# sunshinnnn/DSMnet

Measured on AMD Instinct MI355X. Metric: stereo pairs/sec forward, PSMNet D=192 384×1280, at 1/2/4/8 MI355X, higher is better.
Workload: dtype f32

## Files before the change

### dsmnet_amd/_lib.py

```python
import ctypes
import os

_HERE = os.path.dirname(os.path.abspath(__file__))
LIB_PATH = os.environ.get("DSM_LIB_PATH") or os.path.join(_HERE, "csrc", "libdsmnet_hip.so")

c_int, c_void_p, c_size_t = ctypes.c_int, ctypes.c_void_p, ctypes.c_size_t

DSM_OK = 0
DSM_F32 = 0
DSM_NCDHW, DSM_NDHWC = 0, 1
DSM_CONV_FP32_MFMA, DSM_CONV_COUT1_CHUNKED, DSM_CONV_TM_SHIFT, DSM_CONV_BLOCKS_SHIFT = 1, 2, 4, 16
DSM_CONV_NO_NSPLIT = 4
DSM_CONV_NO_ONCE = 8
DSM_CONV_KSPLIT_SHIFT = 8
DSM_PREC_F32, DSM_PREC_F16, DSM_PREC_F16X2 = 0, 1, 2
DSM_SIM_DOT, DSM_SIM_COSINE = 0, 1
DSM_CORR_BWD_NAIVE = 1


class Bn3dArgs(ctypes.Structure):
    _fields_ = [("y", c_void_p), ("residual", c_void_p), ("out", c_void_p), ("gamma", c_void_p),
                ("beta", c_void_p), ("running_mean", c_void_p), ("running_var", c_void_p),
                ("affine", c_void_p), ("workspace", c_void_p), ("gout", c_void_p), ("dy", c_void_p),
                ("dresidual", c_void_p), ("B", c_int), ("C", c_int),
# ... 138 lines not shown
    "dsm_stage_images_nhwc16": (c_int, [c_void_p] * 3 + [c_int] * 4 + [c_void_p]),
    "dsm_volume_relayout": (c_int, [c_void_p] * 2 + [c_int] * 6 + [c_void_p]),
    "dsm_conv_packed_weight_bytes": (ctypes.c_size_t, [c_int] * 4),
    "dsm_spp_branch_floats": (ctypes.c_size_t, [c_int] * 3),
    "dsm_spp_pool8": (c_int, [c_void_p] * 2 + [c_int] * 3 + [c_void_p]),
    "dsm_spp_branches": (c_int, [c_void_p] * 5 + [c_int] * 3 + [c_void_p]),
    "dsm_spp_concat": (c_int, [c_void_p] * 4 + [c_int] * 3 + [c_void_p] * 2),
    "dsm_warp_abs_error": (c_int, [c_void_p] * 4 + [c_int] * 6 + [ctypes.c_float, c_void_p]),
    "dsm_warp_abs_error_bwd": (c_int, [c_void_p] * 7 + [c_int] * 6 + [ctypes.c_float, c_void_p]),
    "dsm_decoder_cat_bwd": (c_int, [c_void_p] * 6 + [c_int] * 11 + [c_void_p]),
    "dsm_selfsup_workspace_floats": (c_size_t, [ctypes.POINTER(SelfsupItem), c_int]),
    "dsm_selfsup_fwd": (c_int, [ctypes.POINTER(SelfsupItem), c_int, c_int] + [c_void_p] * 4),
    "dsm_selfsup_bwd": (c_int, [ctypes.POINTER(SelfsupItem), c_int, c_int] + [c_void_p] * 4),
    "dsm_selfsup_ext_workspace_floats": (c_size_t, [ctypes.POINTER(SelfsupItem), c_int, c_int]),
    "dsm_selfsup_ext_fwd": (c_int, [ctypes.POINTER(SelfsupItem), ctypes.POINTER(SelfsupExt), c_int, c_int] + [c_void_p] * 4),
    "dsm_selfsup_ext_bwd": (c_int, [ctypes.POINTER(SelfsupItem), ctypes.POINTER(SelfsupExt), c_int, c_int] + [c_void_p] * 4),
    "dsm_selfsup_dyn_fwd": (c_int, [ctypes.POINTER(SelfsupItem), ctypes.POINTER(SelfsupExt), c_int, c_int] + [c_void_p] * 5),
    "dsm_selfsup_dyn_bwd": (c_int, [ctypes.POINTER(SelfsupItem), ctypes.POINTER(SelfsupExt), c_int, c_int] + [c_void_p] * 5),
    "dsm_suploss_workspace_floats": (c_size_t, [c_int] * 5),
    "dsm_suploss_fwd": (c_int, [ctypes.POINTER(SuplossItem), c_int, c_void_p, c_int, c_int, c_int, c_int] + [c_void_p] * 4),
    "dsm_suploss_bwd": (c_int, [ctypes.POINTER(SuplossItem), c_int, c_void_p, c_int, c_int, c_int] + [c_void_p] * 4),
    "dsm_stereo_metrics_workspace_bytes": (c_size_t, [c_int] * 3),
    "dsm_stereo_metrics": (c_int, [ctypes.POINTER(MetricsArgs), c_void_p]),
    "dsm_lr_check": (c_int, [ctypes.POINTER(LrcheckArgs), c_void_p]),
    "dsm_fill_background_workspace_bytes": (c_size_t, [c_int] * 3),
    "dsm_fill_background": (c_int, [c_void_p] * 4 + [c_int] * 3 + [c_void_p]),
    "dsm_stereo_color": (c_int, [c_void_p, c_void_p, ctypes.POINTER(ColorRecord)] + [c_int] * 6 + [c_void_p]),
    "dsm_stereo_spatial": (c_int, [c_void_p, c_void_p, ctypes.POINTER(SpatialRecord)] + [c_int] * 8 + [c_void_p]),
    "dsm_stereo_spatial_raw": (c_int, [c_void_p, c_size_t, ctypes.POINTER(FrameSource), c_void_p,
                                       ctypes.POINTER(SpatialRecord)] + [c_int] * 8 + [c_void_p]),
    "dsm_stereo_spatial_raw_plan": (c_int, [c_void_p, c_size_t, ctypes.POINTER(FrameSource), c_void_p,
                                            ctypes.POINTER(SpatialRecord)] + [c_int] * 8),
    "dsm_concat_conv_fwd": (c_int, [c_void_p] * 5 + [c_size_t] + [c_void_p] * 2 + [c_int] * 9 + [c_void_p]),
}

_lib = None


class DsmnetHipError(RuntimeError):
    pass


def _bind_torch_hip_runtime():
    import torch
    hip = os.path.join(os.path.dirname(torch.__file__), "lib", "libamdhip64.so")
    if os.path.exists(hip):
        ctypes.CDLL(hip, mode=ctypes.RTLD_GLOBAL)


def load():
    global _lib
    if _lib is not None:
        return _lib
    if not os.path.exists(LIB_PATH):
        raise DsmnetHipError(
            "libdsmnet_hip.so not found at %s -- build it with "
            "`python -m dsmnet_amd.csrc.build` (there is no CPU fallback)" % LIB_PATH)
    _bind_torch_hip_runtime()
    lib = ctypes.CDLL(LIB_PATH)
    for name, (res, args) in SIGNATURES.items():
        fn = getattr(lib, name)
        fn.restype = res
        fn.argtypes = args
    if lib.dsm_abi_version() != 7:
        raise DsmnetHipError("libdsmnet_hip.so ABI version mismatch")
    _lib = lib
# ... 8 lines not shown
```

### dsmnet_amd/blocks2d.py

```python
import torch
import torch.nn as nn
import torch.nn.functional as F

from . import costvolume as cv
from . import blocks3d
from .folds import _bump_running_stats, _versions, fold_affine

_TRAIN_2D_MODE = __import__("os").environ.get("DSM_TRAIN_2D", "auto")
_FUSED_TRAIN_2D = _TRAIN_2D_MODE in ("auto", "fused", "conv")
_FUSED_TRAIN_2D_BN = _TRAIN_2D_MODE == "fused"
_TRAIN_2D_MIN_PIXELS = int(__import__("os").environ.get("DSM_TRAIN_2D_MIN_PIXELS", 65536)) if _TRAIN_2D_MODE == "auto" else 0


class own_kernels_only(object):

    def __enter__(self):
        global _TRAIN_2D_MIN_PIXELS, _FUSED_TRAIN_2D
        self.saved = (_TRAIN_2D_MIN_PIXELS, _FUSED_TRAIN_2D)
        _TRAIN_2D_MIN_PIXELS, _FUSED_TRAIN_2D = 0, True
        return self

    def __exit__(self, *exc):
        global _TRAIN_2D_MIN_PIXELS, _FUSED_TRAIN_2D
        _TRAIN_2D_MIN_PIXELS, _FUSED_TRAIN_2D = self.saved
# ... 56 lines not shown
    if not (cv.get_option("wide_conv2d_train") and isinstance(act, nn.ReLU) and isinstance(conv, nn.Conv2d) and
            x.is_cuda and x.dtype == torch.float32):
        return False
    k, s, d, p = conv.kernel_size, conv.stride, conv.dilation, conv.padding
    if k != (3, 3) or s[0] != s[1] or s[0] not in (1, 2) or d != (1, 1) or p != (1, 1) or conv.groups != 1:
        return False
    if conv.bias is None or conv.padding_mode != "zeros" or conv.weight.dtype != torch.float32:
        return False
    if conv.in_channels not in cv.WIDE2D_COUT or conv.out_channels not in cv.WIDE2D_COUT:
        return False
    B, _, H, W = x.shape
    Ho, Wo = (H - 1) // s[0] + 1, (W - 1) // s[0] + 1
    if W > 2032 or B * H * W >= 2 ** 20 or 4 * B * Ho * Wo * conv.out_channels >= 2 ** 31:
        return False
    return _wide_ok(conv, x)


class _Folded2d(object):
    def __init__(self):
        self.key = None
        self.packed = self.scale = self.shift = None

    def get(self, conv, bn, cin_padded):
        srcs = [conv.weight, conv.bias]
        if bn is not None:
            srcs += [bn.weight, bn.bias, bn.running_mean, bn.running_var]
        key = _versions(*srcs) + (cin_padded,)
        if key != self.key:
            with torch.no_grad():
                self.packed = cv.pack_conv2d_weight(conv.weight, cin_padded)
                self.scale, self.shift = fold_affine(conv.bias, bn, conv.out_channels, conv.weight.device)
            self.key = key
        return self.packed, self.scale, self.shift


def train_ok(conv, x):
    if not (_FUSED_TRAIN_2D and isinstance(conv, nn.Conv2d) and torch.is_tensor(x) and x.is_cuda and
            x.dtype == torch.float32 and conv.weight.dtype == torch.float32):
        return False
    k, s, d, p = conv.kernel_size, conv.stride, conv.dilation, conv.padding
    if k[0] != k[1] or s[0] != s[1] or d[0] != d[1] or p[0] != p[1] or conv.groups != 1:
        return False
    if conv.bias is not None or conv.padding_mode != "zeros" or p[0] != d[0] * (k[0] // 2):
        return False
    if x.shape[0] * ((x.shape[2] - 1) // s[0] + 1) * ((x.shape[3] - 1) // s[0] + 1) < _TRAIN_2D_MIN_PIXELS:
        return False
    return x.shape[1] == conv.in_channels and cv.conv2d_variant(conv.out_channels, s[0], k[0], d[0])


def _run_conv2d_autograd(conv, bn, x, residual, relu):
    y = cv.conv2d(x, conv.weight, conv.stride[0], conv.dilation[0])
    if (bn is not None and bn.training and _FUSED_TRAIN_2D_BN and blocks3d._FUSED_TRAIN_BN and
            y.shape[1] % 4 == 0 and y.shape[1] <= 256):
        momentum = bn.momentum if bn.momentum is not None else 0.1
        out = cv.bn_add_relu2d(y, bn.weight, bn.bias, residual,
                               bn.running_mean if bn.track_running_stats else None,
                               bn.running_var if bn.track_running_stats else None,
                               1 if relu else 0, momentum, bn.eps)
        if bn.num_batches_tracked is not None:
            bn.num_batches_tracked += 1
        _bump_running_stats(bn)
        return out
    if bn is not None:
        y = bn(y)
    if residual is not None:
        y = y + residual
# ... 53 lines not shown
```

### dsmnet_amd/costvolume.py

```python
import collections
import ctypes
import functools
import os
import weakref

import torch

from . import _lib
from .folds import _versions

_CL3D = torch.channels_last_3d


class LaunchTimer(object):

    def __init__(self):
        self.records = []

    def start(self):
        ev = torch.cuda.Event(enable_timing=True)
        ev.record()
        return ev

    def stop(self, name, start, work):
# ... 401 lines not shown
            setattr(a, field, 16)
    buf = ctypes.create_string_buffer(96)
    rc = _lib.load().dsm_conv3d_plan(ctypes.byref(a), buf, 96)
    return rc, buf.value.decode()


_PRECISIONS = ("bf16x3", "fp32", "f16x2", "f16")


def _env_precision():
    v = os.environ.get("DSM_CONV_PRECISION", "")
    if v and v not in _PRECISIONS:
        raise ValueError("DSM_CONV_PRECISION must be one of %s, got %r" % (_PRECISIONS, v))
    return v or "f16x2"


def _env_flag(name, default):
    v = os.environ.get(name, "")
    if v not in ("", "0", "1"):
        raise ValueError("%s must be 0 or 1, got %r" % (name, v))
    return default if v == "" else v == "1"


_WIDE_CONV2D_DEFAULT = False

_OPTIONS = {"fuse_volume": True, "fuse_blocks": True, "conv_precision": _env_precision(), "conv_flags": 0,
            "separable_volume": _env_flag("DSM_SEPARABLE_VOLUME", True), "separable_flags": 0,
            "fused_supervised_loss": _env_flag("DSM_FUSED_SUP_LOSS", True),
            "wide_conv2d": _env_flag("DSM_WIDE_CONV2D", _WIDE_CONV2D_DEFAULT),
            "wide_conv2d_train": _env_flag("DSM_WIDE_CONV2D_TRAIN", False),
            "conv2d_k5": _env_flag("DSM_CONV2D_K5", False),
            "warp_train": _env_flag("DSM_WARP_TRAIN", False),
            "decoder_train": _env_flag("DSM_DECODER_TRAIN", False),
            "corr1d_tiled_bwd": False}


def set_option(name, value):
    if name == "conv_fp32":
        old = _OPTIONS["conv_precision"] == "fp32"
        _OPTIONS["conv_precision"] = "fp32" if value else "bf16x3"
        return old
    if name not in _OPTIONS:
        raise KeyError(name)
    old = _OPTIONS[name]
    if name == "conv_precision":
        if value not in _PRECISIONS:
            raise ValueError("conv_precision must be one of %s" % (_PRECISIONS,))
        _OPTIONS[name] = value
    else:
        _OPTIONS[name] = int(value) if name in ("conv_flags", "separable_flags") else bool(value)
    return old


def _mode(mode):
    return _OPTIONS["conv_precision"] if mode is None else mode


def _conv_flags(mode=None):
    return (_lib.DSM_CONV_FP32_MFMA if _mode(mode) == "fp32" else 0) | _OPTIONS["conv_flags"]


def get_option(name):
    if name == "conv_fp32":
        return _OPTIONS["conv_precision"] == "fp32"
    return _OPTIONS[name]

# ... 623 lines not shown
        if needs_amax():
            dy._dsm_amax = _ARENA.slot(y.device)
            a.dy_amax = dy._dsm_amax.data_ptr()
            if dres is not None:
                dres._dsm_amax = _ARENA.slot(y.device)
                a.dres_amax = dres._dsm_amax.data_ptr()
        with torch.cuda.device(y.device), _timed("bn3d_train_bwd_kernels", 4.0 * (3 * y.numel() + gout.numel())):
            rc = _lib.load().dsm_bn3d_train_bwd(ctypes.byref(a), _stream())
        _lib.check(rc, "dsm_bn3d_train_bwd")
        dbeta = ws[:C].float() if has_beta else None
        dgamma = ws[C:].float() if has_gamma else None
        return dy, dgamma, dbeta, dres, None, None, None, None, None


def bn_add_relu3d(y, gamma, beta, residual, running_mean, running_var, relu, momentum, eps):
    return BnAddRelu3dFunction.apply(y, gamma, beta, residual, running_mean, running_var, int(relu),
                                     float(momentum), float(eps))


def stage_images_nhwc16(left, right=None):
    _require_device("stage_images_nhwc16", left, right)
    left = left.contiguous()
    B, C, H, W = left.shape
    if right is not None:
        if tuple(right.shape) != tuple(left.shape):
            raise ValueError("stage_images_nhwc16: the two views differ in shape")
        right = right.contiguous()
    out = torch.empty(((1 if right is None else 2) * B, 16, H, W), device=left.device,
                      dtype=torch.float32, memory_format=_CL2D)
    with torch.cuda.device(left.device):
        rc = _lib.load().dsm_stage_images_nhwc16(_p(left), _p(right), _p(out), B, C, H, W, _stream())
    _lib.check(rc, "dsm_stage_images_nhwc16")
    return out


def conv2d_variant(cout, stride, k, dilation):
    if cout not in (32, 64, 128) or k not in (1, 3) or stride < 1 or dilation < 1:
        return False
    return _conv2d_variant(cout, stride, k, dilation, _mode(None), _conv_flags())


@functools.lru_cache(maxsize=None)
def _conv2d_variant(cout, stride, k, dilation, mode, flags):
    return _conv_plan(_conv2d_standin(1, 16, cout, 12, 40, stride, k, dilation, mode, flags))[0] == _lib.DSM_OK


def _wgrad2d(x_cl, g_cl, stride, dilation, label="conv2d_wgrad_kernel", mode=None):
    B, cx, Hx, Wx = x_cl.shape
    _, cg, Hg, Wg = g_cl.shape
    ws = torch.empty((cx // 32) * (cg // 32) * 9 * 1024, device=x_cl.device, dtype=torch.float32)
    dw = torch.empty((cg, cx, 3, 3), device=x_cl.device, dtype=torch.float32)
    prec, xa, ga = _wgrad_precision(x_cl, g_cl, mode)
    with torch.cuda.device(x_cl.device), _timed(label, 18.0 * cx * cg * B * Hg * Wg):
        rc = _lib.load().dsm_conv2d_wgrad(_p(x_cl), _p(g_cl), _p(ws), _p(dw), B, cx, cg, Hx, Wx,
                                          Hg, Wg, int(stride), int(dilation), _conv_flags(mode), prec,
                                          _p(xa), _p(ga), _stream())
    _lib.check(rc, "dsm_conv2d_wgrad")
    return dw


class Conv2dFunction(torch.autograd.Function):

    @staticmethod
    def forward(ctx, x, weight, stride, dilation):
        _require_device("Conv2dFunction", x, weight)
        cout, cin, k, _ = weight.shape
# ... 785 lines not shown
```

### dsmnet_amd/csrc/build.py

```python
import glob
import os
import subprocess
import sys
from concurrent.futures import ThreadPoolExecutor

HERE = os.path.dirname(os.path.abspath(__file__))
SOURCES = ["abi.hip", "corr1d.hip", "cost_volume.hip", "soft_argmin.hip", "conv3d.hip", "conv_f16.hip",
           "conv3d_bwd.hip", "bn3d.hip", "decoder.hip", "spp.hip", "warp.hip",
           "selfsup.hip", "color.hip", "spatial.hip", "frames.hip", "sepvol.hip", "suploss.hip", "relu_bwd.hip",
           "metrics.hip", "lrcheck.hip"]
LIB = os.path.join(HERE, "libdsmnet_hip.so")
HIPCC = os.environ.get("HIPCC", "/opt/rocm/bin/hipcc")
FLAGS = ["--offload-arch=gfx950", "-O3", "-std=c++17", "-fPIC",
         "-Wall", "-Wno-unused-function"] + os.environ.get("HIPCC_EXTRA", "").split()


def _stale(out, deps):
    if not os.path.exists(out):
        return True
    t = os.path.getmtime(out)
    return any(os.path.getmtime(d) > t for d in deps)


def build(force=False, verbose=True, stamps=False):
    if stamps:
        lib = os.path.join(HERE, "libdsmnet_hip_stamps.so")
        srcs = [os.path.join(HERE, s) for s in SOURCES]
        extra = ["-DDSM_ABLATE=%s" % os.environ["DSM_ABLATE"]] if os.environ.get("DSM_ABLATE") else []
        cmd = [HIPCC] + FLAGS + ["-DDSM_STAMPS"] + extra + ["-shared", "-o", lib] + srcs
        print(" ".join(cmd), flush=True)
        subprocess.run(cmd, check=True)
        return lib
    hdrs = sorted(glob.glob(os.path.join(HERE, "*.hpp"))) + [os.path.join(HERE, "..", "..", "include", "dsmnet_hip.h")]
    srcs = [os.path.join(HERE, s) for s in SOURCES if os.path.exists(os.path.join(HERE, s))]
    objs = []
    jobs = []
    for s in srcs:
        o = s[:-4] + ".o"
        objs.append(o)
        if force or _stale(o, [s] + hdrs):
            jobs.append([HIPCC] + FLAGS + ["-c", s, "-o", o])

    def run(cmd):
# ... 18 lines not shown
```

### dsmnet_amd/models/psmnet/stackhourglass.py

```python
import math

import torch
import torch.nn as nn

from ... import costvolume as cv
from ...blocks3d import Chain3d, ConvBN3d
from .submodule import convbn_3d, disparityregression, feature_extraction


def myadd_3d(tensor1, tensor2):
    assert tensor1.dim() == 5
    d, h, w = (min(a, b) for a, b in zip(tensor1.shape[2:], tensor2.shape[2:]))
    return tensor1[:, :, :d, :h, :w] + tensor2[:, :, :d, :h, :w]


def _deconvbn_3d(cin, cout):
    return ConvBN3d(nn.ConvTranspose3d(cin, cout, kernel_size=3, padding=1, output_padding=1,
                                       stride=2, bias=False), nn.BatchNorm3d(cout))


class hourglass(nn.Module):
    def __init__(self, inplanes):
        super(hourglass, self).__init__()
        c = inplanes
# ... 18 lines not shown
        super(PSMNet, self).__init__()
        self.name = "psmnet"
        self.maxdisp = maxdisp
        self.align_corners = bool(align_corners)
        self.count_levels = 1
        self.feature_extraction = feature_extraction(align_corners=align_corners)
        relu = lambda: nn.ReLU(inplace=True)
        self.dres0 = Chain3d(convbn_3d(64, 32, 3, 1, 1), relu(), convbn_3d(32, 32, 3, 1, 1), relu())
        self.dres1 = Chain3d(convbn_3d(32, 32, 3, 1, 1), relu(), convbn_3d(32, 32, 3, 1, 1))
        self.dres2 = hourglass(32)
        self.dres3 = hourglass(32)
        self.dres4 = hourglass(32)
        for i in (1, 2, 3):
            setattr(self, "classif%d" % i, Chain3d(
                convbn_3d(32, 32, 3, 1, 1), relu(),
                nn.Conv3d(32, 1, kernel_size=3, padding=1, stride=1, bias=False)))
        self._init_weights()

    def _init_weights(self):
        for m in self.modules():
            if isinstance(m, (nn.Conv2d, nn.Conv3d)):
                fan = m.out_channels
                for k in m.kernel_size:
                    fan *= k
                m.weight.data.normal_(0, math.sqrt(2.0 / fan))
            elif isinstance(m, (nn.BatchNorm2d, nn.BatchNorm3d)):
                m.weight.data.fill_(1)
                m.bias.data.zero_()

    def features(self, left, right):
        if self.training:
            return self.feature_extraction(left), self.feature_extraction(right)
        fe = self.feature_extraction
        if left.is_cuda and not torch.is_grad_enabled() and left.shape[1] <= 16:
            both = fe(cv.stage_images_nhwc16(left, right), staged=True)
        else:
            both = self.feature_extraction(torch.cat([left, right], dim=0))
        self.__dict__["_both"] = both
        return (cv.carry_amax(both[: left.shape[0]], both), cv.carry_amax(both[left.shape[0]:], both))

    def regularise(self, cost):
        cost0 = self.dres0(cost)
        cost0 = self.dres1(cost0, residual=cost0)
        out1, pre1, post1 = self.dres2(cost0, None, None, skip=cost0)
        out2, pre2, post2 = self.dres3(out1, pre1, post1, skip=cost0)
        out3, pre3, post3 = self.dres4(out2, pre1, post2, skip=cost0)
        cost1 = self.classif1(out1)
        cost2 = self.classif2(out2, residual=cost1)
        cost3 = self.classif3(out3, residual=cost2)
        return cost1, cost2, cost3

    def forward(self, left, right, mode="train"):
        with cv.amax_scope(left.device):
            return self._forward(left, right)

    def _forward(self, left, right):
        self.__dict__["_both"] = None
        refimg_fea, targetimg_fea = self.features(left, right)
        both = self.__dict__.pop("_both")
        if (both is not None and cv.get_option("fuse_volume") and not torch.is_grad_enabled() and
                cv.virtual_volume_ok(both.shape[1])):
            cost = cv.VirtualVolume(both, self.maxdisp // 4, True)
        else:
            cost = cv.concat_volume(refimg_fea, targetimg_fea, self.maxdisp // 4, mask_left=True)
        size = (self.maxdisp, left.shape[2], left.shape[3])
        cost1, cost2, cost3 = self.regularise(cost)
        pred1 = cv.soft_argmin(cost1, size, align_corners=self.align_corners)
# ... 4 lines not shown
```

### dsmnet_amd/models/psmnet/submodule.py

```python
import torch
import torch.nn as nn
import torch.nn.functional as F

from ... import blocks2d
from ... import costvolume as cv
from ...blocks2d import ConvBN2d, _Folded2d, run_conv2d, stage_image_nhwc16
from ...blocks3d import ConvBN3d
from ...folds import _versions, fold_affine

_SPP_MATMUL = __import__("os").environ.get("DSM_TRAIN_SPP", "matmul") != "interp"
_TRAIN_NHWC = __import__("os").environ.get("DSM_TRAIN_LAYOUT", "nchw") == "nhwc"


def convbn(in_planes, out_planes, kernel_size, stride, pad, dilation):
    del pad
    return ConvBN2d(
        nn.Conv2d(in_planes, out_planes, kernel_size=kernel_size, stride=stride,
                  padding=dilation, dilation=dilation, bias=False),
        nn.BatchNorm2d(out_planes))


def convbn_3d(in_planes, out_planes, kernel_size, stride, pad):
    conv = nn.Conv3d(in_planes, out_planes, kernel_size=kernel_size, padding=pad,
                     stride=stride, bias=False)
    return ConvBN3d(conv, nn.BatchNorm3d(out_planes))


class BasicBlock(nn.Module):
    expansion = 1

    def __init__(self, inplanes, planes, stride, downsample, pad, dilation):
        super(BasicBlock, self).__init__()
        self.conv1 = nn.Sequential(convbn(inplanes, planes, 3, stride, pad, dilation),
                                   nn.ReLU(inplace=True))
        self.conv2 = convbn(planes, planes, 3, 1, pad, dilation)
        self.downsample = downsample
        self.stride = stride

    def forward(self, x):
        fused = blocks2d.run_basicblock(self.conv1[0], self.conv2, x, self.downsample)
        if fused is not None:
            return fused
        y = self.conv1[0](x, relu=True)
        skip = x if self.downsample is None else self.downsample(x)
        return self.conv2(y, residual=skip)


class disparityregression(nn.Module):

    def __init__(self, maxdisp):
        super(disparityregression, self).__init__()
        self.maxdisp = maxdisp

    def forward(self, x):
        return cv.soft_argmin(torch.log(x.clamp_min(1e-38)), None, negate=False)


class feature_extraction(nn.Module):

    def __init__(self, align_corners=False):
        super(feature_extraction, self).__init__()
        self.align_corners = bool(align_corners)
        self.inplanes = 32
        stem = []
        for cin, stride in ((3, 2), (32, 1), (32, 1)):
            stem += [convbn(cin, 32, 3, stride, 1, 1), nn.ReLU(inplace=True)]
        self.firstconv = nn.Sequential(*stem)
        self.layer1 = self._make_layer(BasicBlock, 32, 3, 1, 1, 1)
        self.layer2 = self._make_layer(BasicBlock, 64, 16, 2, 1, 1)
        self.layer3 = self._make_layer(BasicBlock, 128, 3, 1, 1, 1)
        self.layer4 = self._make_layer(BasicBlock, 128, 3, 1, 1, 2)
        for idx, pool in ((1, 64), (2, 32), (3, 16), (4, 8)):
            setattr(self, "branch%d" % idx, nn.Sequential(
                nn.AvgPool2d((pool, pool), stride=(pool, pool)),
                convbn(128, 32, 1, 1, 0, 1), nn.ReLU(inplace=True)))
        self.lastconv = nn.Sequential(
            convbn(320, 128, 3, 1, 1, 1), nn.ReLU(inplace=True),
            nn.Conv2d(128, 32, kernel_size=1, padding=0, stride=1, bias=False))

    def _make_layer(self, block, planes, blocks, stride, pad, dilation):
        downsample = None
        if stride != 1 or self.inplanes != planes * block.expansion:
            downsample = ConvBN2d(
                nn.Conv2d(self.inplanes, planes * block.expansion, kernel_size=1,
                          stride=stride, bias=False),
                nn.BatchNorm2d(planes * block.expansion))
        layers = [block(self.inplanes, planes, stride, downsample, pad, dilation)]
        self.inplanes = planes * block.expansion
        layers += [block(self.inplanes, planes, 1, None, pad, dilation) for _ in range(1, blocks)]
        return nn.Sequential(*layers)

    @staticmethod
    def _bilinear_matrix(n_in, n_out, align_corners, device):
        i = torch.arange(n_out, dtype=torch.float32, device=device)
        if align_corners:
            src = i * ((n_in - 1) / (n_out - 1)) if n_out > 1 else torch.zeros_like(i)
        else:
            src = ((i + 0.5) * (n_in / n_out) - 0.5).clamp_min(0.0)
        i0 = src.floor().long().clamp_max(n_in - 1)
        i1 = (i0 + 1).clamp_max(n_in - 1)
        w1 = src - i0.to(src.dtype)
        m = torch.zeros((n_out, n_in), dtype=torch.float32, device=device)
        m.scatter_add_(1, i0[:, None], (1.0 - w1)[:, None])
        m.scatter_add_(1, i1[:, None], w1[:, None])
# ... 4 lines not shown
            return F.interpolate(y, size=size, mode="bilinear", align_corners=self.align_corners)
        key = (y.shape[2], y.shape[3], size[0], size[1], self.align_corners, y.device)
        cache = self.__dict__.setdefault("_up_cache", {})
        if key not in cache:
            cache[key] = (self._bilinear_matrix(y.shape[2], size[0], self.align_corners, y.device),
                          self._bilinear_matrix(y.shape[3], size[1], self.align_corners, y.device).t().contiguous())
        ry, rxt = cache[key]
        return torch.matmul(ry, torch.matmul(y.contiguous(), rxt))

    def _spp_stock(self, raw, skip):
        size = skip.shape[2:]
        pooled, pyramid = skip, []
        for i in (4, 3, 2, 1):
            pooled = F.avg_pool2d(pooled, 8 if i == 4 else 2)
            branch = getattr(self, "branch%d" % i)
            y = branch[1](pooled, relu=True)
            pyramid.append(self._upsample(y, size))
        return torch.cat([raw, skip] + pyramid, dim=1)

    def _spp_params(self):
        convs = [getattr(self, "branch%d" % i)[1] for i in (4, 3, 2, 1)]
        srcs = [t for c in convs for t in (c[0].weight, c[1].weight, c[1].bias,
                                           c[1].running_mean, c[1].running_var)]
        key = _versions(*srcs)
        if getattr(self, "_spp_key", None) != key:
            with torch.no_grad():
                w_t = torch.stack([c[0].weight.reshape(32, 128).t() for c in convs]).contiguous()
                rows = [fold_affine(None, c[1], 32, c[0].weight.device) for c in convs]
                scale, shift = (torch.stack(r) for r in zip(*rows))
            self._spp_cache = (w_t, scale, shift)
            self._spp_key = key
        return self._spp_cache

    def forward(self, x, staged=False):
        fast = x.is_cuda and not self.training and not torch.is_grad_enabled()
        if staged and not fast:
            raise RuntimeError("feature_extraction: staged input exists on the eval fast path only")
        if fast and not staged:
            x = stage_image_nhwc16(x)
        elif _TRAIN_NHWC and x.is_cuda:
            x = x.contiguous(memory_format=torch.channels_last)
        x = self.firstconv[0](x, relu=True)
        fc2, fc4 = self.firstconv[2], self.firstconv[4]
        y = blocks2d.run_basicblock_layers(fc2._folded, fc2[0], fc2[1], fc4._folded, fc4[0], fc4[1], x, True, skip=False)
        x = y if y is not None else fc4(fc2(x, relu=True), relu=True)
        x = self.layer1(x)
        raw = self.layer2(x)
        skip = self.layer4(self.layer3(raw))
        if skip.is_cuda and not self.training and not torch.is_grad_enabled() and not self.align_corners:
            x = cv.spp_head(raw, skip, *self._spp_params())
        else:
            x = self._spp_stock(raw, skip)
        x = self.lastconv[0](x, relu=True)
        if not hasattr(self, "_last_fold"):
            self._last_fold = _Folded2d()
        return run_conv2d(self._last_fold, self.lastconv[2], None, x)
```

### include/dsmnet_hip.h

```cpp
#ifndef DSMNET_HIP_H
#define DSMNET_HIP_H

#include <stddef.h>
#include <stdint.h>

#ifdef __cplusplus
extern "C" {
#endif

#define DSM_ABI_VERSION 7

#define DSM_OK               0
#define DSM_ERR_ARG         -1
#define DSM_ERR_UNSUPPORTED -2
#define DSM_ERR_LAUNCH      -3
#define DSM_ERR_ALIGN       -4

enum dsm_dtype  { DSM_F32 = 0 };
enum dsm_layout { DSM_NCDHW = 0, DSM_NDHWC = 1 };

typedef void* dsm_stream_t;

int         dsm_abi_version(void);
const char* dsm_strerror(int code);
// ... 330 lines not shown
  double scale_x, scale_y;
} dsm_spatial_record;

int dsm_stereo_spatial(const void* x, void* y, const dsm_spatial_record* recs, int n_recs, int B, int C,
                       int H0, int W0, int h, int w, int to_tensor_channels, dsm_stream_t stream);

#define DSM_DISP_F32 0
#define DSM_DISP_U16_256 1
#define DSM_DISP_U16 2
#define DSM_DISP_U8 3
#define DSM_FRAMES_MAX_RECORDS 32
typedef struct dsm_frame_source {
  long long imL, imR;
  long long dispL, dispR;
  int Hs, Ws;
  int y0, x0;
  int flip;
  int disp_format;
  int pad_[2];
} dsm_frame_source;

int dsm_stereo_spatial_raw(const void* raw, size_t raw_bytes, const dsm_frame_source* srcs, void* y,
                           const dsm_spatial_record* recs, int n_recs, int B, int C, int H0, int W0, int h,
                           int w, int to_tensor_channels, dsm_stream_t stream);
int dsm_stereo_spatial_raw_plan(const void* raw, size_t raw_bytes, const dsm_frame_source* srcs, void* y,
                                const dsm_spatial_record* recs, int n_recs, int B, int C, int H0, int W0,
                                int h, int w, int to_tensor_channels);

int dsm_concat_conv_fwd(const void* both, const void* w_packed, const void* scale, const void* shift,
                        void* workspace, size_t workspace_floats, void* y, float* y_amax,
                        int B, int C, int Cout, int D, int H, int W,
                        int mask_left, int relu, int flags, dsm_stream_t stream);

#ifdef __cplusplus
}
#endif
#endif
```

Measured before the change: 207.4.

## Add dedicated MFMA kernels for the feature-tower stem conv and 1x1 convs

Adds a stem kernel that reads the raw left and right NCHW images directly and computes the 3->32 stride-2 3x3 conv with fp32 MFMA plus the folded BN and ReLU. This skips the separate NHWC16 staging pass and the padded-channel conv. It also adds a 1x1 pointwise MFMA kernel for the downsample projections in layer2/layer3 and for the final lastconv. Both paths are on by default under a new option, at the cost of extra weight-packing code and specialised kernels.

After: 209.1, median of 4. No clear change (+0.8%).

```diff
diff --git a/dsmnet_amd/_lib.py b/dsmnet_amd/_lib.py
--- a/dsmnet_amd/_lib.py
+++ b/dsmnet_amd/_lib.py
@@ -194,6 +194,8 @@
     "dsm_stereo_spatial_raw_plan": (c_int, [c_void_p, c_size_t, ctypes.POINTER(FrameSource), c_void_p,
                                             ctypes.POINTER(SpatialRecord)] + [c_int] * 8),
     "dsm_concat_conv_fwd": (c_int, [c_void_p] * 5 + [c_size_t] + [c_void_p] * 2 + [c_int] * 9 + [c_void_p]),
+    "dsm_conv2d_stem_fwd": (c_int, [c_void_p] * 7 + [c_int] * 5 + [c_void_p]),
+    "dsm_conv2d_pointwise_fwd": (c_int, [c_void_p] * 6 + [c_int] * 8 + [c_void_p]),
 }
 
 _lib = None
diff --git a/dsmnet_amd/blocks2d.py b/dsmnet_amd/blocks2d.py
--- a/dsmnet_amd/blocks2d.py
+++ b/dsmnet_amd/blocks2d.py
@@ -112,6 +112,55 @@
                 self.scale, self.shift = fold_affine(conv.bias, bn, conv.out_channels, conv.weight.device)
             self.key = key
         return self.packed, self.scale, self.shift
+
+
+class _FoldedSmall(object):
+
+    def __init__(self, pack):
+        self.pack, self.key = pack, None
+        self.packed = self.scale = self.shift = None
+
+    def get(self, conv, bn):
+        srcs = [conv.weight, conv.bias]
+        if bn is not None:
+            srcs += [bn.weight, bn.bias, bn.running_mean, bn.running_var]
+        key = _versions(*srcs)
+        if key != self.key:
+            with torch.no_grad():
+                self.packed = self.pack(conv.weight)
+                self.scale, self.shift = fold_affine(conv.bias, bn, conv.out_channels, conv.weight.device)
+            self.key = key
+        return self.packed, self.scale, self.shift
+
+
+def _small_ok(conv, bn, x):
+    return (cv.get_option("tower_small_ops") and isinstance(conv, nn.Conv2d) and torch.is_tensor(x) and x.is_cuda and
+            x.dtype == torch.float32 and x.dim() == 4 and conv.weight.dtype == torch.float32 and
+            not torch.is_grad_enabled() and not (bn is not None and bn.training) and conv.groups == 1 and
+            conv.padding_mode == "zeros" and x.shape[1] == conv.in_channels)
+
+
+def stem_ok(conv, bn, x):
+    return (_small_ok(conv, bn, x) and conv.in_channels == 3 and conv.out_channels == 32 and
+            conv.kernel_size == (3, 3) and conv.stride == (2, 2) and conv.padding == (1, 1) and conv.dilation == (1, 1))
+
+
+def run_stem(folded, conv, bn, left, right=None, relu=True):
+    packed, scale, shift = folded.get(conv, bn)
+    return cv.conv2d_stem(left, right, packed, scale, shift, relu=relu)
+
+
+def pointwise_ok(conv, bn, x):
+    return (_small_ok(conv, bn, x) and conv.kernel_size == (1, 1) and conv.stride in ((1, 1), (2, 2)) and
+            conv.padding == (0, 0) and conv.dilation == (1, 1) and conv.in_channels in cv.POINTWISE_CHANNELS and
+            conv.out_channels in cv.POINTWISE_CHANNELS)
+
+
+def run_pointwise(folded, conv, bn, x, relu=False):
+    packed, scale, shift = folded.get(conv, bn)
+    if not x.is_contiguous(memory_format=cv._CL2D):
+        x = cv.carry_amax(x.contiguous(memory_format=cv._CL2D), x)
+    return cv.conv2d_pointwise(x, packed, conv.out_channels, scale, shift, stride=conv.stride[0], relu=relu)
 
 
 def train_ok(conv, x):
diff --git a/dsmnet_amd/costvolume.py b/dsmnet_amd/costvolume.py
--- a/dsmnet_amd/costvolume.py
+++ b/dsmnet_amd/costvolume.py
@@ -457,6 +457,7 @@
             "conv2d_k5": _env_flag("DSM_CONV2D_K5", False),
             "warp_train": _env_flag("DSM_WARP_TRAIN", False),
             "decoder_train": _env_flag("DSM_DECODER_TRAIN", False),
+            "tower_small_ops": _env_flag("DSM_TOWER_SMALL_OPS", True),
             "corr1d_tiled_bwd": False}
 
 
@@ -1146,6 +1147,81 @@
         rc = _lib.load().dsm_stage_images_nhwc16(_p(left), _p(right), _p(out), B, C, H, W, _stream())
     _lib.check(rc, "dsm_stage_images_nhwc16")
     return out
+
+
+POINTWISE_CHANNELS = (32, 64, 128)
+
+
+def pack_conv2d_stem_weight(weight):
+    if tuple(weight.shape) != (32, 3, 3, 3):
+        raise ValueError("pack_conv2d_stem_weight: expected (32, 3, 3, 3), got %s" % (tuple(weight.shape),))
+    w = weight.detach().to(torch.float32).reshape(32, 9, 3)
+    first = w[:, :, :2].permute(1, 2, 0)
+    last = torch.cat([w[:, :, 2], w.new_zeros(32, 1)], dim=1).reshape(32, 5, 2).permute(1, 2, 0)
+    return torch.cat([first, last], dim=0).contiguous().reshape(-1)
+
+
+def pack_conv2d_pointwise_weight(weight):
+    if weight.dim() != 4 or tuple(weight.shape[2:]) != (1, 1):
+        raise ValueError("pack_conv2d_pointwise_weight: expected (Cout, Cin, 1, 1), got %s" % (tuple(weight.shape),))
+    cout, cin = weight.shape[:2]
+    if cin not in POINTWISE_CHANNELS or cout not in POINTWISE_CHANNELS:
+        raise ValueError("pack_conv2d_pointwise_weight: Cin and Cout must be 32, 64 or 128, got %d -> %d" % (cin, cout))
+    w = weight.detach().to(torch.float32).reshape(cout // 32, 32, 2, cin // 2)
+    return w.permute(0, 3, 2, 1).contiguous().reshape(-1)
+
+
+def conv2d_stem(left, right, packed_weight, scale=None, shift=None, relu=True, grid=0):
+    _require_device("conv2d_stem", left, right, packed_weight, scale, shift)
+    if left.dim() != 4 or left.shape[1] != 3:
+        raise ValueError("conv2d_stem: expected (B, 3, H, W) images, got %s" % (tuple(left.shape),))
+    if right is not None and tuple(right.shape) != tuple(left.shape):
+        raise ValueError("conv2d_stem: the two views differ in shape")
+    if packed_weight.numel() != 14 * 2 * 32:
+        raise ValueError("conv2d_stem: packed weight has %d floats, expected %d" % (packed_weight.numel(), 14 * 2 * 32))
+    left = left.contiguous()
+    if right is not None:
+        right = right.contiguous()
+    B, _, H, W = left.shape
+    nB = B if right is None else 2 * B
+    Ho, Wo = (H - 1) // 2 + 1, (W - 1) // 2 + 1
+    y = torch.empty((nB, 32, Ho, Wo), device=left.device, dtype=torch.float32, memory_format=_CL2D)
+    ya = _ARENA.slot(y.device) if needs_amax() else None
+    work = 4.0 * (nB * 3 * H * W + y.numel())
+    with torch.cuda.device(left.device), _timed("conv2d_stem_kernel", work):
+        rc = _lib.load().dsm_conv2d_stem_fwd(_p(left), _p(right), _p(packed_weight), _p(scale), _p(shift), _p(y),
+                                             _p(ya), B, H, W, int(bool(relu)), int(grid), _stream())
+    _lib.check(rc, "dsm_conv2d_stem_fwd")
+    if ya is not None:
+        y._dsm_amax = ya
+    return y
+
+
+def conv2d_pointwise(x, packed_weight, cout, scale=None, shift=None, stride=1, relu=False, grid=0):
+    _require_device("conv2d_pointwise", x, packed_weight, scale, shift)
+    if x.dim() != 4 or not x.is_contiguous(memory_format=_CL2D):
+        raise ValueError("conv2d_pointwise: expected a (B, C, H, W) map in channels_last memory, got shape %s, "
+                         "strides %s" % (tuple(x.shape), tuple(x.stride())))
+    B, cin, Hi, Wi = x.shape
+    stride = int(stride)
+    if stride < 1:
+        raise ValueError("conv2d_pointwise: stride must be positive, got %d" % stride)
+    if packed_weight.numel() != cin * cout:
+        raise ValueError("conv2d_pointwise: packed weight has %d floats, expected %d" % (packed_weight.numel(), cin * cout))
+    for name, t in (("scale", scale), ("shift", shift)):
+        if t is not None and t.numel() != cout:
+            raise ValueError("conv2d_pointwise: %s has %d floats, expected %d" % (name, t.numel(), cout))
+    Ho, Wo = (Hi - 1) // stride + 1, (Wi - 1) // stride + 1
+    y = torch.empty((B, cout, Ho, Wo), device=x.device, dtype=torch.float32, memory_format=_CL2D)
+    ya = _ARENA.slot(y.device) if needs_amax() else None
+    work = 4.0 * (B * Ho * Wo * cin + cin * cout + y.numel())
+    with torch.cuda.device(x.device), _timed("conv2d_pointwise_kernel", work):
+        rc = _lib.load().dsm_conv2d_pointwise_fwd(_p(x), _p(packed_weight), _p(scale), _p(shift), _p(y), _p(ya),
+                                                  B, cin, cout, Hi, Wi, stride, int(bool(relu)), int(grid), _stream())
+    _lib.check(rc, "dsm_conv2d_pointwise_fwd")
+    if ya is not None:
+        y._dsm_amax = ya
+    return y
 
 
 def conv2d_variant(cout, stride, k, dilation):
diff --git a/dsmnet_amd/csrc/build.py b/dsmnet_amd/csrc/build.py
--- a/dsmnet_amd/csrc/build.py
+++ b/dsmnet_amd/csrc/build.py
@@ -8,7 +8,7 @@
 SOURCES = ["abi.hip", "corr1d.hip", "cost_volume.hip", "soft_argmin.hip", "conv3d.hip", "conv_f16.hip",
            "conv3d_bwd.hip", "bn3d.hip", "decoder.hip", "spp.hip", "warp.hip",
            "selfsup.hip", "color.hip", "spatial.hip", "frames.hip", "sepvol.hip", "suploss.hip", "relu_bwd.hip",
-           "metrics.hip", "lrcheck.hip"]
+           "metrics.hip", "lrcheck.hip", "tower_small.hip"]
 LIB = os.path.join(HERE, "libdsmnet_hip.so")
 HIPCC = os.environ.get("HIPCC", "/opt/rocm/bin/hipcc")
 FLAGS = ["--offload-arch=gfx950", "-O3", "-std=c++17", "-fPIC",
diff --git a/dsmnet_amd/csrc/tower_small.hip b/dsmnet_amd/csrc/tower_small.hip
--- /dev/null
+++ b/dsmnet_amd/csrc/tower_small.hip
@@ -0,0 +1,260 @@
+#include "split_core.hpp"
+
+namespace {
+
+constexpr int TS_THREADS = 256;
+constexpr int TS_PIX = 32;
+constexpr int TS_CUS = 256;
+
+constexpr int STEM_STEPS = 14;
+constexpr int STEM_CO = 32;
+constexpr int STEM_SUB = 2;
+
+struct StemParams {
+  const float* left; const float* right; const float* wp;
+  const float* scale; const float* shift;
+  float* y; float* y_amax;
+  int B, H, W, Ho, Wo, tpr, ntiles, relu;
+};
+
+__global__ __launch_bounds__(TS_THREADS) __attribute__((amdgpu_waves_per_eu(4)))
+void conv2d_stem_kernel(StemParams p) {
+  __shared__ float red[4];
+  const int lane = threadIdx.x & 63, wave = __builtin_amdgcn_readfirstlane(threadIdx.x >> 6);
+  const int pl = lane & 31, h = lane >> 5;
+  float w[STEM_STEPS];
+#pragma unroll
+  for (int j = 0; j < STEM_STEPS; ++j) w[j] = p.wp[j * 64 + lane];
+  const float sc = p.scale ? p.scale[pl] : 1.f, sh = p.shift ? p.shift[pl] : 0.f;
+  const int plane = p.H * p.W;
+  float am = 0.f;
+  for (int tile = blockIdx.x * 4 + wave; tile < p.ntiles; tile += gridDim.x * 4) {
+    const int xt = tile % p.tpr, row = tile / p.tpr;
+    const int yo = row % p.Ho, n = row / p.Ho;
+    const float* img = n < p.B ? p.left + (long)n * 3 * plane : p.right + (long)(n - p.B) * 3 * plane;
+    float a[STEM_SUB][STEM_STEPS];
+#pragma unroll
+    for (int s = 0; s < STEM_SUB; ++s) {
+      const int xo = (xt * STEM_SUB + s) * TS_PIX + pl;
+      const int xb = 2 * xo - 1;
+      const bool col_h = xo < p.Wo && xb + h >= 0 && xb + h < p.W;
+      const bool col_2 = xo < p.Wo && xb + 2 < p.W;
+#pragma unroll
+      for (int j = 0; j < 9; ++j) {
+        const int yy = 2 * yo + j % 3 - 1;
+        const bool ok = col_h && yy >= 0 && yy < p.H;
+        const float v = img[ok ? (j / 3) * plane + yy * p.W + xb + h : 0];
+        a[s][j] = ok ? v : 0.f;
+      }
+#pragma unroll
+      for (int j = 9; j < STEM_STEPS; ++j) {
+        const int r0 = 2 * (j - 9), r1 = r0 + 1;
+        const int y0 = 2 * yo + r0 % 3 - 1, y1 = 2 * yo + r1 % 3 - 1;
+        const bool ok0 = y0 >= 0 && y0 < p.H, ok1 = r1 < 9 && y1 >= 0 && y1 < p.H;
+        const int o0 = (r0 / 3) * plane + y0 * p.W, o1 = (r1 / 3) * plane + y1 * p.W;
+        const bool ok = col_2 && (h ? ok1 : ok0);
+        const float v = img[ok ? (h ? o1 : o0) + xb + 2 : 0];
+        a[s][j] = ok ? v : 0.f;
+      }
+    }
+    __builtin_amdgcn_sched_barrier(0);
+    f32x16 acc[STEM_SUB];
+#pragma unroll
+    for (int s = 0; s < STEM_SUB; ++s)
+      acc[s] = f32x16{0.f, 0.f, 0.f, 0.f, 0.f, 0.f, 0.f, 0.f, 0.f, 0.f, 0.f, 0.f, 0.f, 0.f, 0.f, 0.f};
+#pragma unroll
+    for (int j = 0; j < STEM_STEPS; ++j) {
+#pragma unroll
+      for (int s = 0; s < STEM_SUB; ++s) acc[s] = __builtin_amdgcn_mfma_f32_32x32x2f32(a[s][j], w[j], acc[s], 0, 0, 0);
+    }
+#pragma unroll
+    for (int s = 0; s < STEM_SUB; ++s) {
+      const int x0 = (xt * STEM_SUB + s) * TS_PIX;
+      float* dst = p.y + ((long)row * p.Wo + x0) * STEM_CO + pl;
+#pragma unroll
+      for (int r = 0; r < 16; ++r) {
+        const int px = (r & 3) + 8 * (r >> 2) + 4 * h;
+        if (x0 + px < p.Wo) {
+          float v = acc[s][r] * sc + sh;
+          if (p.relu) v = fmaxf(v, 0.f);
+          am = fmaxf(am, fabsf(v));
+          dst[(long)px * STEM_CO] = v;
+        }
+      }
+    }
+  }
+  publish_amax<4, false>(p.y_amax, am, red);
+}
+
+struct PwParams {
+  const float* x; const float* wp; const float* scale; const float* shift;
+  float* y; float* y_amax;
+  long NP;
+  int Hi, Wi, Ho, Wo, stride, ntiles, relu;
+};
+
+template <int CIN>
+__device__ __forceinline__ void pw_load(const PwParams& p, int tile, int pl, int h, f32x4 (&a)[CIN / 8]) {
+  const long g = (long)tile * TS_PIX + pl;
+  const bool ok = g < p.NP;
+  long ip = ok ? g : 0;
+  if (p.stride != 1) {
+    const int xo = (int)(ip % p.Wo);
+    const long t = ip / p.Wo;
+    const int yo = (int)(t % p.Ho);
+    ip = ((t / p.Ho) * p.Hi + (long)yo * p.stride) * p.Wi + (long)xo * p.stride;
+  }
+  const f32x4* src = reinterpret_cast<const f32x4*>(p.x + ip * CIN + h * (CIN / 2));
+#pragma unroll
+  for (int q = 0; q < CIN / 8; ++q) a[q] = ok ? src[q] : f32x4{0.f, 0.f, 0.f, 0.f};
+}
+
+constexpr int pw_waves(int cin, int cout) {
+  const int need = cin + cout / 2 + cout / 4 + 32;
+  return need <= 80 ? 6 : need <= 96 ? 5 : need <= 128 ? 4 : need <= 168 ? 3 : 2;
+}
+
+template <int CIN, int COUT>
+__global__ __launch_bounds__(TS_THREADS) __attribute__((amdgpu_waves_per_eu(pw_waves(CIN, COUT))))
+void conv2d_pointwise_kernel(PwParams p) {
+  constexpr int KS = CIN / 2, NB = COUT / 32;
+  extern __shared__ __align__(16) float lds[];
+  float* wl = lds;
+  float* red = lds + CIN * COUT;
+  const int lane = threadIdx.x & 63, wave = __builtin_amdgcn_readfirstlane(threadIdx.x >> 6);
+  const int pl = lane & 31, h = lane >> 5;
+  const int step = gridDim.x * 4;
+  int tile = blockIdx.x * 4 + wave;
+
+  f32x4 cur[CIN / 8], pre[CIN / 8];
+  pw_load<CIN>(p, tile, pl, h, cur);
+  for (int i = threadIdx.x; i < CIN * COUT / 4; i += TS_THREADS)
+    reinterpret_cast<f32x4*>(wl)[i] = reinterpret_cast<const f32x4*>(p.wp)[i];
+  float sc[NB], sh[NB];
+#pragma unroll
+  for (int ob = 0; ob < NB; ++ob) {
+    sc[ob] = p.scale ? p.scale[ob * 32 + pl] : 1.f;
+    sh[ob] = p.shift ? p.shift[ob * 32 + pl] : 0.f;
+  }
+  __syncthreads();
+
+  float am = 0.f;
+  for (; tile < p.ntiles; tile += step) {
+    const bool more = tile + step < p.ntiles;
+    if (more) pw_load<CIN>(p, tile + step, pl, h, pre);
+    f32x16 acc[NB];
+#pragma unroll
+    for (int ob = 0; ob < NB; ++ob)
+      acc[ob] = f32x16{0.f, 0.f, 0.f, 0.f, 0.f, 0.f, 0.f, 0.f, 0.f, 0.f, 0.f, 0.f, 0.f, 0.f, 0.f, 0.f};
+    float b[2][4 * NB];
+#pragma unroll
+    for (int i = 0; i < 4 * NB; ++i) b[0][i] = wl[((i / 4) * KS + (i & 3)) * 64 + lane];
+#pragma unroll
+    for (int q = 0; q < KS / 4; ++q) {
+      if (q + 1 < KS / 4) {
+#pragma unroll
+        for (int i = 0; i < 4 * NB; ++i) b[(q + 1) & 1][i] = wl[((i / 4) * KS + 4 * (q + 1) + (i & 3)) * 64 + lane];
+      }
+#pragma unroll
+      for (int jj = 0; jj < 4; ++jj) {
+#pragma unroll
+        for (int ob = 0; ob < NB; ++ob)
+          acc[ob] = __builtin_amdgcn_mfma_f32_32x32x2f32(cur[q][jj], b[q & 1][ob * 4 + jj], acc[ob], 0, 0, 0);
+      }
+      __builtin_amdgcn_sched_barrier(0);
+    }
+    const long g0 = (long)tile * TS_PIX;
+    float* dst = p.y + g0 * COUT + pl;
+#pragma unroll
+    for (int r = 0; r < 16; ++r) {
+      const int px = (r & 3) + 8 * (r >> 2) + 4 * h;
+      if (g0 + px < p.NP) {
+#pragma unroll
+        for (int ob = 0; ob < NB; ++ob) {
+          float v = acc[ob][r] * sc[ob] + sh[ob];
+          if (p.relu) v = fmaxf(v, 0.f);
+          am = fmaxf(am, fabsf(v));
+          dst[(long)px * COUT + ob * 32] = v;
+        }
+      }
+    }
+    if (more) {
+#pragma unroll
+      for (int q = 0; q < CIN / 8; ++q) cur[q] = pre[q];
+    }
+  }
+  publish_amax<4, false>(p.y_amax, am, red);
+}
+
+template <int CIN, int COUT>
+int pw_launch(const PwParams& p, int grid, hipStream_t s) {
+  constexpr size_t lds = (size_t)CIN * COUT * 4 + 16;
+  if (lds > 64 * 1024) DSM_REQUIRE((dsm_allow_lds<conv2d_pointwise_kernel<CIN, COUT>>(lds) == DSM_OK), DSM_ERR_LAUNCH);
+  hipLaunchKernelGGL((conv2d_pointwise_kernel<CIN, COUT>), dim3((unsigned)grid), dim3(TS_THREADS), lds, s, p);
+  return dsm_launch_status();
+}
+
+template <int CIN>
+int pw_launch_cout(const PwParams& p, int Cout, int grid, hipStream_t s) {
+  switch (Cout) {
+    case 32: return pw_launch<CIN, 32>(p, grid, s);
+    case 64: return pw_launch<CIN, 64>(p, grid, s);
+    default: return pw_launch<CIN, 128>(p, grid, s);
+  }
+}
+
+int ts_grid(int ntiles, int grid, int per_cu) {
+  const int need = dsm_cdiv(ntiles, 4);
+  if (grid <= 0) grid = TS_CUS * per_cu;
+  return grid < need ? grid : need;
+}
+
+}
+
+extern "C" int dsm_conv2d_stem_fwd(const void* left, const void* right, const void* w_packed, const void* scale,
+                                   const void* shift, void* y, float* y_amax, int B, int H, int W, int relu,
+                                   int grid, dsm_stream_t stream) {
+  DSM_REQUIRE(left && w_packed && y, DSM_ERR_ARG);
+  DSM_REQUIRE(B >= 1 && H >= 1 && W >= 1 && grid >= 0, DSM_ERR_ARG);
+  DSM_REQUIRE(dsm_aligned16(w_packed) && dsm_aligned16(y) && dsm_aligned16(scale) && dsm_aligned16(shift), DSM_ERR_ALIGN);
+  DSM_REQUIRE((((uintptr_t)left | (uintptr_t)right | (uintptr_t)y_amax) & 3u) == 0, DSM_ERR_ALIGN);
+  StemParams p;
+  p.left = (const float*)left; p.right = (const float*)right; p.wp = (const float*)w_packed;
+  p.scale = (const float*)scale; p.shift = (const float*)shift;
+  p.y = (float*)y; p.y_amax = y_amax;
+  p.B = B; p.H = H; p.W = W; p.Ho = (H - 1) / 2 + 1; p.Wo = (W - 1) / 2 + 1;
+  p.tpr = dsm_cdiv(p.Wo, TS_PIX * STEM_SUB);
+  const long nt = (long)(right ? 2 : 1) * B * p.Ho * p.tpr;
+  DSM_REQUIRE(nt < (1L << 30) && 3L * H * W < (1L << 31), DSM_ERR_UNSUPPORTED);
+  p.ntiles = (int)nt; p.relu = relu ? 1 : 0;
+  dsm_clear_stale_error();
+  hipLaunchKernelGGL(conv2d_stem_kernel, dim3((unsigned)ts_grid(p.ntiles, grid, 4)), dim3(TS_THREADS), 0,
+                     (hipStream_t)stream, p);
+  return dsm_launch_status();
+}
+
+extern "C" int dsm_conv2d_pointwise_fwd(const void* x, const void* w_packed, const void* scale, const void* shift,
+                                        void* y, float* y_amax, int B, int Cin, int Cout, int Hi, int Wi,
+                                        int stride, int relu, int grid, dsm_stream_t stream) {
+  DSM_REQUIRE(x && w_packed && y, DSM_ERR_ARG);
+  DSM_REQUIRE(B >= 1 && Cin >= 1 && Cout >= 1 && Hi >= 1 && Wi >= 1 && stride >= 1 && grid >= 0, DSM_ERR_ARG);
+  DSM_REQUIRE(stride <= 2, DSM_ERR_UNSUPPORTED);
+  DSM_REQUIRE((Cin == 32 || Cin == 64 || Cin == 128) && (Cout == 32 || Cout == 64 || Cout == 128), DSM_ERR_UNSUPPORTED);
+  DSM_REQUIRE(dsm_aligned16(x) && dsm_aligned16(w_packed) && dsm_aligned16(y) && dsm_aligned16(scale) &&
+              dsm_aligned16(shift) && (((uintptr_t)y_amax) & 3u) == 0, DSM_ERR_ALIGN);
+  PwParams p;
+  p.x = (const float*)x; p.wp = (const float*)w_packed; p.scale = (const float*)scale; p.shift = (const float*)shift;
+  p.y = (float*)y; p.y_amax = y_amax;
+  p.Hi = Hi; p.Wi = Wi; p.Ho = (Hi - 1) / stride + 1; p.Wo = (Wi - 1) / stride + 1;
+  p.NP = (long)B * p.Ho * p.Wo;
+  DSM_REQUIRE(p.NP < (1L << 30) * TS_PIX, DSM_ERR_UNSUPPORTED);
+  p.stride = stride; p.ntiles = dsm_cdiv(p.NP, TS_PIX); p.relu = relu ? 1 : 0;
+  const int g = ts_grid(p.ntiles, grid, 4);
+  hipStream_t s = (hipStream_t)stream;
+  dsm_clear_stale_error();
+  switch (Cin) {
+    case 32: return pw_launch_cout<32>(p, Cout, g, s);
+    case 64: return pw_launch_cout<64>(p, Cout, g, s);
+    default: return pw_launch_cout<128>(p, Cout, g, s);
+  }
+}
diff --git a/dsmnet_amd/models/psmnet/stackhourglass.py b/dsmnet_amd/models/psmnet/stackhourglass.py
--- a/dsmnet_amd/models/psmnet/stackhourglass.py
+++ b/dsmnet_amd/models/psmnet/stackhourglass.py
@@ -74,7 +74,9 @@
         if self.training:
             return self.feature_extraction(left), self.feature_extraction(right)
         fe = self.feature_extraction
-        if left.is_cuda and not torch.is_grad_enabled() and left.shape[1] <= 16:
+        if right.shape == left.shape and fe.stem_from_images(left) and fe.stem_from_images(right):
+            both = fe(left, right=right)
+        elif left.is_cuda and not torch.is_grad_enabled() and left.shape[1] <= 16:
             both = fe(cv.stage_images_nhwc16(left, right), staged=True)
         else:
             both = self.feature_extraction(torch.cat([left, right], dim=0))
diff --git a/dsmnet_amd/models/psmnet/submodule.py b/dsmnet_amd/models/psmnet/submodule.py
--- a/dsmnet_amd/models/psmnet/submodule.py
+++ b/dsmnet_amd/models/psmnet/submodule.py
@@ -28,6 +28,7 @@
 
 class BasicBlock(nn.Module):
     expansion = 1
+    small_ops = False
 
     def __init__(self, inplanes, planes, stride, downsample, pad, dilation):
         super(BasicBlock, self).__init__()
@@ -42,7 +43,15 @@
         if fused is not None:
             return fused
         y = self.conv1[0](x, relu=True)
-        skip = x if self.downsample is None else self.downsample(x)
+        ds = self.downsample
+        if ds is None:
+            skip = x
+        elif self.small_ops and isinstance(ds, ConvBN2d) and blocks2d.pointwise_ok(ds[0], ds[1], x):
+            if "_ds_fold" not in self.__dict__:
+                self.__dict__["_ds_fold"] = blocks2d._FoldedSmall(cv.pack_conv2d_pointwise_weight)
+            skip = blocks2d.run_pointwise(self._ds_fold, ds[0], ds[1], x)
+        else:
+            skip = ds(x)
         return self.conv2(y, residual=skip)
 
 
@@ -70,6 +79,7 @@
         self.layer2 = self._make_layer(BasicBlock, 64, 16, 2, 1, 1)
         self.layer3 = self._make_layer(BasicBlock, 128, 3, 1, 1, 1)
         self.layer4 = self._make_layer(BasicBlock, 128, 3, 1, 1, 2)
+        self.layer2[0].small_ops = self.layer3[0].small_ops = True
         for idx, pool in ((1, 64), (2, 32), (3, 16), (4, 8)):
             setattr(self, "branch%d" % idx, nn.Sequential(
                 nn.AvgPool2d((pool, pool), stride=(pool, pool)),
@@ -140,15 +150,31 @@
             self._spp_key = key
         return self._spp_cache
 
-    def forward(self, x, staged=False):
+    def _fold(self, name, pack):
+        if name not in self.__dict__:
+            self.__dict__[name] = blocks2d._FoldedSmall(pack)
+        return self.__dict__[name]
+
+    def stem_from_images(self, x):
+        fc0 = self.firstconv[0]
+        return not self.training and blocks2d.stem_ok(fc0[0], fc0[1], x)
+
+    def forward(self, x, staged=False, right=None):
         fast = x.is_cuda and not self.training and not torch.is_grad_enabled()
         if staged and not fast:
             raise RuntimeError("feature_extraction: staged input exists on the eval fast path only")
-        if fast and not staged:
-            x = stage_image_nhwc16(x)
-        elif _TRAIN_NHWC and x.is_cuda:
-            x = x.contiguous(memory_format=torch.channels_last)
-        x = self.firstconv[0](x, relu=True)
+        stem = fast and not staged and self.stem_from_images(x)
+        if right is not None and not stem:
+            raise RuntimeError("feature_extraction: a second view exists where the stem reads the images only")
+        if stem:
+            fc0 = self.firstconv[0]
+            x = blocks2d.run_stem(self._fold("_stem_fold", cv.pack_conv2d_stem_weight), fc0[0], fc0[1], x, right)
+        else:
+            if fast and not staged:
+                x = stage_image_nhwc16(x)
+            elif _TRAIN_NHWC and x.is_cuda:
+                x = x.contiguous(memory_format=torch.channels_last)
+            x = self.firstconv[0](x, relu=True)
         fc2, fc4 = self.firstconv[2], self.firstconv[4]
         y = blocks2d.run_basicblock_layers(fc2._folded, fc2[0], fc2[1], fc4._folded, fc4[0], fc4[1], x, True, skip=False)
         x = y if y is not None else fc4(fc2(x, relu=True), relu=True)
@@ -160,6 +186,9 @@
         else:
             x = self._spp_stock(raw, skip)
         x = self.lastconv[0](x, relu=True)
+        if not self.training and blocks2d.pointwise_ok(self.lastconv[2], None, x):
+            return blocks2d.run_pointwise(self._fold("_last_small_fold", cv.pack_conv2d_pointwise_weight),
+                                          self.lastconv[2], None, x)
         if not hasattr(self, "_last_fold"):
             self._last_fold = _Folded2d()
         return run_conv2d(self._last_fold, self.lastconv[2], None, x)
diff --git a/include/dsmnet_hip.h b/include/dsmnet_hip.h
--- a/include/dsmnet_hip.h
+++ b/include/dsmnet_hip.h
@@ -386,6 +386,13 @@
                         int B, int C, int Cout, int D, int H, int W,
                         int mask_left, int relu, int flags, dsm_stream_t stream);
 
+int dsm_conv2d_stem_fwd(const void* left, const void* right, const void* w_packed, const void* scale,
+                        const void* shift, void* y, float* y_amax, int B, int H, int W, int relu, int grid,
+                        dsm_stream_t stream);
+int dsm_conv2d_pointwise_fwd(const void* x, const void* w_packed, const void* scale, const void* shift,
+                             void* y, float* y_amax, int B, int Cin, int Cout, int Hi, int Wi, int stride,
+                             int relu, int grid, dsm_stream_t stream);
+
 #ifdef __cplusplus
 }
 #endif
```
